# yc015/fully-automated-multi-heartbeat-echocardiography-video-segmentation-and-motion-tracking

Measured on AMD Instinct MI355X. Metric: 32f×112×112 clips/sec at 1/2/4/8 MI355X; Dice Δ vs CPU ref, higher is better.
Workload: dtype fp32

## Files before the change

### fully-automated-multi-heartbeat-echocardiography-video-segmentation-and-motion-tracking_amd/csrc/conv.hip

```cpp
#include <hip/hip_bf16.h>
#include <stdlib.h>
#include <string.h>

#include "common.h"

typedef __bf16 bf16x8 __attribute__((ext_vector_type(8)));

namespace {

__device__ inline bf16x8 pack_bf16x8(f32x4 a, f32x4 b) {
  return bf16x8{(__bf16)a[0], (__bf16)a[1], (__bf16)a[2], (__bf16)a[3],
                (__bf16)b[0], (__bf16)b[1], (__bf16)b[2], (__bf16)b[3]};
}

__device__ inline void split3_bf16x8(f32x4 a, f32x4 b, bf16x8& hi, bf16x8& mid, bf16x8& lo) {
  hi = pack_bf16x8(a, b);
#pragma unroll
  for (int e = 0; e < 4; ++e) {
    a[e] -= (float)hi[e];
    b[e] -= (float)hi[4 + e];
  }
  mid = pack_bf16x8(a, b);
#pragma unroll
  for (int e = 0; e < 4; ++e) {
// ... 916 lines not shown
    }
  };
  auto store_tiles = [&](int buf) {
#pragma unroll
    for (int i = 0; i < AL; ++i) As[buf][a_q[i]][a_r[i]] = ra[i];
#pragma unroll
    for (int i = 0; i < BL; ++i) {
      const int e = tid + i * NTH;
      if (e < B4) Bs[buf][e & 3][e >> 2] = rb[i];
    }
  };
  f32x4 acc[MT][NT];
#pragma unroll
  for (int i = 0; i < MT; ++i)
#pragma unroll
    for (int j = 0; j < NT; ++j) acc[i][j] = f32x4{0.f, 0.f, 0.f, 0.f};
  const int nk = p.Kp / 16;
  load_tiles(0);
  store_tiles(0);
  __syncthreads();
  int cur = 0;
  for (int kt = 0; kt < nk; ++kt) {
    const bool more = kt + 1 < nk;
    if (more) load_tiles((kt + 1) * 16);
    f32x4 a[MT], b[NT];
#pragma unroll
    for (int i = 0; i < MT; ++i) a[i] = As[cur][q][wid * 32 + i * 16 + l16];
#pragma unroll
    for (int j = 0; j < NT; ++j) b[j] = Bs[cur][q][j * 16 + l16];
#pragma unroll
    for (int kk = 0; kk < 4; ++kk)
#pragma unroll
      for (int i = 0; i < MT; ++i)
#pragma unroll
        for (int j = 0; j < NT; ++j)
          acc[i][j] = __builtin_amdgcn_mfma_f32_16x16x4f32(b[j][kk], a[i][kk], acc[i][j], 0, 0, 0);
    if (more) store_tiles(cur ^ 1);
    __syncthreads();
    cur ^= 1;
  }
  epilogue<MT, NT>(p, acc, m0 + wid * 32, n0, q, l16);
}


__device__ inline bf16x8 stem_bf16x8(f32x4 a, f32x4 b) {
  return bf16x8{(__bf16)a[0], (__bf16)a[1], (__bf16)a[2], (__bf16)a[3],
                (__bf16)b[0], (__bf16)b[1], (__bf16)b[2], (__bf16)b[3]};
}

__global__ __launch_bounds__(256) __attribute__((amdgpu_waves_per_eu(2))) void conv_stem_bf16(ConvParams p, int n_items) {
  constexpr int MT = 4, NT = 4, ROW = 7 * 64, IMG = 64 * ROW;
  __shared__ __align__(16) char ws[2 * IMG];
  const float* x = reinterpret_cast<const float*>(p.x);
  const char* w16 = reinterpret_cast<const char*>(p.w);
  const int tid = threadIdx.x, lane = tid & 63, wid = tid >> 6;
  const int q = lane >> 4, l16 = lane & 15;
  const int q8 = n_items >> 3, r8 = n_items & 7, x8 = blockIdx.x & 7;
  const int i_start = x8 < r8 ? x8 * (q8 + 1) : r8 * (q8 + 1) + (x8 - r8) * q8;
  const int i_end = i_start + q8 + (x8 < r8 ? 1 : 0);
  const int i_step = gridDim.x >> 3;
  if (i_start + (int)(blockIdx.x >> 3) >= i_end) return;
  for (int e = tid; e < 2 * 64 * 28; e += 256) {
    const int im = e / (64 * 28), r0 = e - im * (64 * 28);
    const int co = r0 / 28, r = r0 - co * 28, kh = r >> 2, sl = r & 3;
    *reinterpret_cast<uint4*>(ws + im * IMG + co * ROW + kh * 64 + ((sl ^ (co & 3)) << 4)) =
        *reinterpret_cast<const uint4*>(w16 + (size_t)im * 64 * 448 + (size_t)co * 448 + kh * 64 + sl * 16);
  }
  __syncthreads();
  const int b_rd = l16 * ROW + ((q ^ (l16 & 3)) << 4);
  f32x4 bv[NT];
#pragma unroll
  for (int j = 0; j < NT; ++j) bv[j] = *reinterpret_cast<const f32x4*>(p.bias + 16 * j + 4 * q);
#pragma unroll 1
  for (int item = i_start + (int)(blockIdx.x >> 3); item < i_end; item += i_step) {
    const int m0 = item * 256 + wid * 64;
    const float* rowp[MT];
    int hi0[MT], wi0[MT];
    bool live[MT];
#pragma unroll
    for (int i = 0; i < MT; ++i) {
      int m = m0 + 16 * i + l16;
      live[i] = m < p.M;
      if (!live[i]) m = 0;
      const int wo = m % p.Wo;
      m /= p.Wo;
      const int ho = m % p.Ho;
      const int nt = m / p.Ho;
      hi0[i] = 2 * ho - 3;
      wi0[i] = 2 * wo - 3 + 2 * q;
      rowp[i] = x + ((size_t)nt * p.Hi * p.Wi) * 4;
    }
    f32x4 acc[MT][NT];
#pragma unroll
    for (int i = 0; i < MT; ++i)
#pragma unroll
      for (int j = 0; j < NT; ++j) acc[i][j] = f32x4{0.f, 0.f, 0.f, 0.f};
#pragma unroll 1
    for (int kh = 0; kh < 7; ++kh) {
      bf16x8 ah[MT], al[MT], bh[NT], bl[NT];
#pragma unroll
      for (int i = 0; i < MT; ++i) {
        const int hi = hi0[i] + kh;
        const bool rok = live[i] && (unsigned)hi < (unsigned)p.Hi;
        const float* px = rowp[i] + ((size_t)hi * p.Wi + wi0[i]) * 4;
        f32x4 v0 = {0.f, 0.f, 0.f, 0.f}, v1 = {0.f, 0.f, 0.f, 0.f};
        if (rok && (unsigned)wi0[i] < (unsigned)p.Wi) v0 = *reinterpret_cast<const f32x4*>(px);
        if (rok && (unsigned)(wi0[i] + 1) < (unsigned)p.Wi) v1 = *reinterpret_cast<const f32x4*>(px + 4);
        ah[i] = stem_bf16x8(v0, v1);
        f32x4 r0, r1;
#pragma unroll
        for (int e = 0; e < 4; ++e) {
          r0[e] = v0[e] - (float)ah[i][e];
          r1[e] = v1[e] - (float)ah[i][4 + e];
        }
        al[i] = stem_bf16x8(r0, r1);
      }
#pragma unroll
      for (int j = 0; j < NT; ++j) {
        bh[j] = *reinterpret_cast<const bf16x8*>(ws + j * 16 * ROW + kh * 64 + b_rd);
        bl[j] = *reinterpret_cast<const bf16x8*>(ws + IMG + j * 16 * ROW + kh * 64 + b_rd);
      }
#pragma unroll
      for (int j = 0; j < NT; ++j)
#pragma unroll
        for (int i = 0; i < MT; ++i) {
          acc[i][j] = __builtin_amdgcn_mfma_f32_16x16x32_bf16(bl[j], ah[i], acc[i][j], 0, 0, 0);
          acc[i][j] = __builtin_amdgcn_mfma_f32_16x16x32_bf16(bh[j], al[i], acc[i][j], 0, 0, 0);
          acc[i][j] = __builtin_amdgcn_mfma_f32_16x16x32_bf16(bh[j], ah[i], acc[i][j], 0, 0, 0);
        }
    }
    __bf16* y = reinterpret_cast<__bf16*>(p.y);
#pragma unroll
    for (int i = 0; i < MT; ++i) {
      if (!live[i]) continue;
      const size_t m = (size_t)m0 + 16 * i + l16;
#pragma unroll
      for (int j = 0; j < NT; ++j) {
        const int n = 16 * j + 4 * q;
        f32x4 v = acc[i][j] + bv[j];
#pragma unroll
        for (int e = 0; e < 4; ++e) v[e] = relu1(v[e]);
        *reinterpret_cast<bf16x4*>(y + m * 64 + n) = bf16x4{(__bf16)v[0], (__bf16)v[1], (__bf16)v[2], (__bf16)v[3]};
      }
    }
  }
}

bool dma_buf_ok(const ConvParams& p, size_t es) {
  if ((p.vflags & CLASFV_VARIANT_NO_DMA_BUF) || es != 2) return false;
  const size_t lim = (size_t)1 << 31;
  const size_t vox = (size_t)p.N * p.Ti * p.Hi * p.Wi;
  const size_t padpix = ((size_t)p.pt * p.Hi + p.ph) * p.Wi + p.pw;
  return p.KT * p.KH * p.KW <= 32 && (vox + padpix) * p.Cin * es < lim && (!p.x2 || vox * p.Cin2 * es < lim) &&
         (size_t)p.Cout * p.Kp * es < lim;
}

bool dma_w_ok_(const ConvParams& p) {
  if (p.vflags & CLASFV_VARIANT_NO_DMA_W) return false;
  if (!p.in_bf16 || p.stem || p.n_split > 1 || !dma_buf_ok(p, 2)) return false;
  return p.Cin % 64 == 0 && (!p.x2 || p.Cin2 % 64 == 0) && p.Kp == p.K && p.Kp % 64 == 0;
}

template <int MT, int NT, int S>
hipError_t launch_dma_w(const ConvParams& p, hipStream_t s) {
  constexpr int BM = 64 * MT, BN = 16 * NT;
  const int mt = (p.M + BM - 1) / BM, nt = (p.Cout + BN - 1) / BN;
  const DmaDivs dv{fast_div(p.Wo), fast_div(p.Ho), fast_div(p.To), fast_div(nt)};
  CLASFV_LAUNCH((conv_dma_w<MT, NT, S>), dim3(mt * nt), dim3(256), 0, s, p, nt, dv);
  return hipGetLastError();
}

template <typename T, int MT, int NT, int S>
hipError_t launch_dma(const ConvParams& p, hipStream_t s) {
  constexpr int BM = 64 * MT, BN = 16 * NT;
  const int mt = (p.M + BM - 1) / BM, nt = (p.Cout + BN - 1) / BN;
  const DmaDivs dv{fast_div(p.Wo), fast_div(p.Ho), fast_div(p.To), fast_div(nt)};
  const int n_split = p.n_split > 1 ? p.n_split : 1;
  if constexpr (sizeof(T) == 2 && MT == 2)
    if (dma_w_ok_(p)) return launch_dma_w<MT, NT, 2>(p, s);
  if (dma_buf_ok(p, sizeof(T)))
    CLASFV_LAUNCH((conv_dma<T, MT, NT, S, true>), dim3(mt * nt * n_split), dim3(256), 0, s, p, nt, dv);
  else
    CLASFV_LAUNCH((conv_dma<T, MT, NT, S>), dim3(mt * nt * n_split), dim3(256), 0, s, p, nt, dv);
  if (n_split > 1) return launch_split_sum(p, s);
  return hipGetLastError();
}

bool dma_x3_buf_ok(const ConvParams& p, int rows_alloc) {
  if (p.vflags & CLASFV_VARIANT_NO_DMA_BUF) return false;
  const size_t lim = (size_t)1 << 31;
  const size_t vox = (size_t)p.N * p.Ti * p.Hi * p.Wi;
  const size_t padpix = ((size_t)p.pt * p.Hi + p.ph) * p.Wi + p.pw;
  const int npairs = (p.Kp / 16 + 1) / 2;
  return p.KT * p.KH * p.KW <= 31 && (vox + padpix) * p.Cin * 4 < lim && (!p.x2 || vox * p.Cin2 * 4 < lim) &&
         (size_t)rows_alloc * npairs * 192 < lim;
}

template <int MT, int NT, int S, int WN = 1>
hipError_t launch_dma_x3_t(const ConvParams& p, hipStream_t s) {
  constexpr int BM = 64 * MT, BN = 16 * NT;
  const int mt = (p.M + BM - 1) / BM, nt = (p.Cout + BN - 1) / BN;
  const DmaDivs dv{fast_div(p.Wo), fast_div(p.Ho), fast_div(p.To), fast_div(nt)};
  const int n_split = p.n_split > 1 ? p.n_split : 1;
  const dim3 grid(mt * nt * n_split);
  const int ef = n_split > 1 ? 0 : (p.res ? 1 : 0) | (p.relu ? 2 : 0) | (p.y_c8 ? 4 : 0);
  switch (dma_x3_buf_ok(p, nt * BN) ? ef + 8 : ef) {
    case 0: CLASFV_LAUNCH((conv_dma_x3<MT, NT, S, WN, 0>), grid, dim3(256), 0, s, p, nt, dv); break;
    case 1: CLASFV_LAUNCH((conv_dma_x3<MT, NT, S, WN, 1>), grid, dim3(256), 0, s, p, nt, dv); break;
    case 2: CLASFV_LAUNCH((conv_dma_x3<MT, NT, S, WN, 2>), grid, dim3(256), 0, s, p, nt, dv); break;
    case 3: CLASFV_LAUNCH((conv_dma_x3<MT, NT, S, WN, 3>), grid, dim3(256), 0, s, p, nt, dv); break;
    case 8: CLASFV_LAUNCH((conv_dma_x3<MT, NT, S, WN, 0, 0, true>), grid, dim3(256), 0, s, p, nt, dv); break;
    case 9: CLASFV_LAUNCH((conv_dma_x3<MT, NT, S, WN, 1, 0, true>), grid, dim3(256), 0, s, p, nt, dv); break;
    case 10: CLASFV_LAUNCH((conv_dma_x3<MT, NT, S, WN, 2, 0, true>), grid, dim3(256), 0, s, p, nt, dv); break;
    case 11: CLASFV_LAUNCH((conv_dma_x3<MT, NT, S, WN, 3, 0, true>), grid, dim3(256), 0, s, p, nt, dv); break;
    default:
      if (ef >= 8 || ef < 4) return hipErrorInvalidValue;
      if (dma_x3_buf_ok(p, nt * BN))
        CLASFV_LAUNCH((conv_dma_x3<MT, NT, S, WN, -1, 0, true>), grid, dim3(256), 0, s, p, nt, dv);
      else
        CLASFV_LAUNCH((conv_dma_x3<MT, NT, S, WN>), grid, dim3(256), 0, s, p, nt, dv);
      break;
  }
  if (n_split > 1) return launch_split_sum(p, s);
  return hipGetLastError();
}

template <int NT>
hipError_t launch_stem(const ConvParams& p, hipStream_t s) {
  if (p.Cin != 4 || p.KT != 1 || p.KH != 7 || p.KW != 7) return hipErrorInvalidValue;
  const int mt = (p.M + 127) / 128, nt = (p.Cout + 16 * NT - 1) / (16 * NT);
  CLASFV_LAUNCH((conv_stem_f32<NT>), dim3(mt * nt), dim3(256), 0, s, p, nt);
  return hipGetLastError();
}

#ifdef CLASFV_KNOCKOUTS
template <int NT, int KO>
hipError_t dma_ko_t(const ConvParams& p, hipStream_t s) {
  constexpr int BM = 128, BN = 16 * NT;
  const int mt = (p.M + BM - 1) / BM, nt = (p.Cout + BN - 1) / BN;
  const DmaDivs dv{fast_div(p.Wo), fast_div(p.Ho), fast_div(p.To), fast_div(nt)};
  CLASFV_LAUNCH((conv_dma<__bf16, 2, NT, 3, (KO & 1) == 0, KO & ~1>), dim3(mt * nt), dim3(256), 0, s, p, nt, dv);
  return hipGetLastError();
}
template <int NT>
hipError_t dma_ko_n(const ConvParams& p, int ko, hipStream_t s) {
  switch (ko) {
    case 0: return dma_ko_t<NT, 0>(p, s);
    case 1: return dma_ko_t<NT, 1>(p, s);
    case 4: return dma_ko_t<NT, 4>(p, s);
    case 8: return dma_ko_t<NT, 8>(p, s);
    case 16: return dma_ko_t<NT, 16>(p, s);
    case 12: return dma_ko_t<NT, 12>(p, s);
    case 28: return dma_ko_t<NT, 28>(p, s);
  }
  return hipErrorInvalidValue;
}
hipError_t dma_bf16_ko(const ConvParams& p, int bn, int ko, hipStream_t s) {
  if (ko == 100 || ko == 101) {
    if (!dma_w_ok_(p)) return hipErrorInvalidValue;
    switch (bn) {
      case 64: return ko == 100 ? launch_dma_w<2, 4, 2>(p, s) : launch_dma_w<2, 4, 3>(p, s);
      case 96: return ko == 100 ? launch_dma_w<2, 6, 2>(p, s) : launch_dma_w<2, 6, 3>(p, s);
      case 128: return ko == 100 ? launch_dma_w<2, 8, 2>(p, s) : launch_dma_w<2, 8, 3>(p, s);
    }
    return hipErrorInvalidValue;
  }
  if (!p.in_bf16 || p.n_split > 1) return hipErrorInvalidValue;
  switch (bn) {
    case 64: return dma_ko_n<4>(p, ko, s);
    case 96: return dma_ko_n<6>(p, ko, s);
    case 128: return dma_ko_n<8>(p, ko, s);
  }
  return hipErrorInvalidValue;
}
#endif

template <typename T>
hipError_t launch_typed(const ConvParams& p, int bn, hipStream_t s) {
  switch (bn) {
    case 48: return launch_dma<T, 2, 3, 3>(p, s);
    case 64: return launch_dma<T, 2, 4, 3>(p, s);
    case 80: return launch_dma<T, 2, 5, 3>(p, s);
    case 96: return launch_dma<T, 2, 6, 3>(p, s);
    case 128: return launch_dma<T, 2, 8, 3>(p, s);
    case 144: return launch_dma<T, 2, 9, 3>(p, s);
  }
  return hipErrorInvalidValue;
}

#ifdef CLASFV_KNOCKOUTS
hipError_t launch_bf16_m4(const ConvParams& p, int bn, hipStream_t s) {
  switch (bn) {
    case 48: return launch_dma<__bf16, 4, 3, 3>(p, s);
    case 64: return launch_dma<__bf16, 4, 4, 3>(p, s);
    case 80: return launch_dma<__bf16, 4, 5, 3>(p, s);
    case 96: return launch_dma<__bf16, 4, 6, 3>(p, s);
    case 128: return launch_dma<__bf16, 4, 8, 3>(p, s);
    case 144: return launch_dma<__bf16, 4, 9, 3>(p, s);
  }
  return hipErrorInvalidValue;
}
#endif

__global__ __launch_bounds__(256) __attribute__((amdgpu_waves_per_eu(2))) void conv_stem_x3(ConvParams p, int n_items) {
  constexpr int MT = 4, NT = 3, CO = 16 * NT, ROW = 7 * 64, IMG = CO * ROW;
  __shared__ __align__(16) char ws[3 * IMG];
  const float* x = reinterpret_cast<const float*>(p.x);
  const char* w16 = reinterpret_cast<const char*>(p.w);
  const int tid = threadIdx.x, lane = tid & 63, wid = tid >> 6;
  const int q = lane >> 4, l16 = lane & 15;
  const int q8 = n_items >> 3, r8 = n_items & 7, x8 = blockIdx.x & 7;
  const int i_start = x8 < r8 ? x8 * (q8 + 1) : r8 * (q8 + 1) + (x8 - r8) * q8;
  const int i_end = i_start + q8 + (x8 < r8 ? 1 : 0);
  const int i_step = gridDim.x >> 3;
  if (i_start + (int)(blockIdx.x >> 3) >= i_end) return;
  for (int e = tid; e < 3 * CO * 28; e += 256) {
    const int im = e / (CO * 28), r0 = e - im * (CO * 28);
    const int co = r0 / 28, r = r0 - co * 28, kh = r >> 2, sl = r & 3;
    *reinterpret_cast<uint4*>(ws + im * IMG + co * ROW + kh * 64 + ((sl ^ (co & 3)) << 4)) =
        *reinterpret_cast<const uint4*>(w16 + (size_t)im * CO * 448 + (size_t)co * 448 + kh * 64 + sl * 16);
  }
  __syncthreads();
  const int b_rd = l16 * ROW + ((q ^ (l16 & 3)) << 4);
#pragma unroll 1
  for (int item = i_start + (int)(blockIdx.x >> 3); item < i_end; item += i_step) {
  const int m0 = item * 256 + wid * 64;
  const float* rowp[MT];
  int hi0[MT], wi0[MT];
  bool live[MT];
#pragma unroll
  for (int i = 0; i < MT; ++i) {
    int m = m0 + 16 * i + l16;
    live[i] = m < p.M;
    if (!live[i]) m = 0;
    const int wo = m % p.Wo;
    m /= p.Wo;
    const int ho = m % p.Ho;
    const int nt = m / p.Ho;
    hi0[i] = 2 * ho - 3;
    wi0[i] = 2 * wo - 3 + 2 * q;
    rowp[i] = x + ((size_t)nt * p.Hi * p.Wi) * 4;
  }
  f32x4 acc[MT][NT];
#pragma unroll
  for (int i = 0; i < MT; ++i)
#pragma unroll
    for (int j = 0; j < NT; ++j) acc[i][j] = f32x4{0.f, 0.f, 0.f, 0.f};
#pragma unroll 1
  for (int kh = 0; kh < 7; ++kh) {
    bf16x8 ah[MT], am[MT], al[MT];
#pragma unroll
    for (int i = 0; i < MT; ++i) {
      const int hi = hi0[i] + kh;
      const bool rok = live[i] && (unsigned)hi < (unsigned)p.Hi;
      const float* px = rowp[i] + ((size_t)hi * p.Wi + wi0[i]) * 4;
      f32x4 v0 = {0.f, 0.f, 0.f, 0.f}, v1 = {0.f, 0.f, 0.f, 0.f};
      if (rok && (unsigned)wi0[i] < (unsigned)p.Wi) v0 = *reinterpret_cast<const f32x4*>(px);
      if (rok && (unsigned)(wi0[i] + 1) < (unsigned)p.Wi) v1 = *reinterpret_cast<const f32x4*>(px + 4);
      split3_bf16x8(v0, v1, ah[i], am[i], al[i]);
    }
#pragma unroll
    for (int j = 0; j < NT; ++j) {
      const bf16x8 bh = *reinterpret_cast<const bf16x8*>(ws + j * 16 * ROW + kh * 64 + b_rd);
      const bf16x8 bm = *reinterpret_cast<const bf16x8*>(ws + IMG + j * 16 * ROW + kh * 64 + b_rd);
      const bf16x8 bl = *reinterpret_cast<const bf16x8*>(ws + 2 * IMG + j * 16 * ROW + kh * 64 + b_rd);
#pragma unroll
      for (int i = 0; i < MT; ++i) {
        f32x4 c = acc[i][j];
        c = __builtin_amdgcn_mfma_f32_16x16x32_bf16(bl, ah[i], c, 0, 0, 0);
        c = __builtin_amdgcn_mfma_f32_16x16x32_bf16(bh, al[i], c, 0, 0, 0);
        c = __builtin_amdgcn_mfma_f32_16x16x32_bf16(bm, am[i], c, 0, 0, 0);
        c = __builtin_amdgcn_mfma_f32_16x16x32_bf16(bm, ah[i], c, 0, 0, 0);
        c = __builtin_amdgcn_mfma_f32_16x16x32_bf16(bh, am[i], c, 0, 0, 0);
        acc[i][j] = __builtin_amdgcn_mfma_f32_16x16x32_bf16(bh, ah[i], c, 0, 0, 0);
      }
    }
  }
  epilogue<MT, NT>(p, acc, m0, 0, q, l16);
  }
}

}

bool dma_w_ok(const ConvParams& p) { return dma_w_ok_(p); }

#ifdef CLASFV_KNOCKOUTS
hipError_t launch_dma_bf16_ko(const ConvParams& p, int bn, int ko, hipStream_t s) { return dma_bf16_ko(p, bn, ko, s); }
#endif

bool proj_x3_supported(const ConvParams& p) {
  if (p.vflags & CLASFV_VARIANT_NO_DMA_X3) return false;
  if (p.in_bf16 || p.out_bf16 || p.stem || p.x_c8 || p.y_c8 || p.n_split > 1) return false;
  if (p.KT != 1 || p.KH != 1 || p.KW != 1 || p.st != 1 || p.sh != 1 || p.sw != 1) return false;
  if (p.Cout != 64 || p.Cin % 32 || (p.x2 && p.Cin2 % 32)) return false;
  const int k = p.Cin + (p.x2 ? p.Cin2 : 0);
  if (p.Kp != k || k != 128) return false;
  return (size_t)p.M * (p.Cin > 64 ? p.Cin : 64) < ((size_t)1 << 31);
}

hipError_t launch_proj_x3(const ConvParams& p, hipStream_t s) {
  if (!proj_x3_supported(p)) return hipErrorInvalidValue;
  const int n_items = (p.M + 31) / 32;
  const int kb = p.Kp / 32;
  int blocks = 256;
  if (blocks * 4 > n_items) blocks = (n_items + 3) / 4;
  (void)kb;
  const int passes = (n_items + 4 * blocks - 1) / (4 * blocks);
  CLASFV_LAUNCH_P(passes, (conv_proj_x3<4, 3>), dim3(blocks), dim3(256), 0, s, p, n_items);
  return hipGetLastError();
}

bool dma_x3_supported(const ConvParams& p) {
  return !(p.vflags & CLASFV_VARIANT_NO_DMA_X3) && !p.in_bf16 && !p.out_bf16 && !p.stem && !p.x_c8 && !p.y_c8 &&
         p.Kp % 16 == 0 && p.Cin % 16 == 0 && (!p.x2 || p.Cin2 % 16 == 0) && p.Cout % 16 == 0;
}

int dma_x3_bn(int cout_p) {
  const int n16 = cout_p / 16;
  for (int c : {8, 6, 5, 4, 3})
    if (n16 % c == 0) return 16 * c;
  return 16 * (n16 % 2 == 0 ? 2 : 1);
}

hipError_t launch_dma_x3(const ConvParams& p, int bn, hipStream_t s) {
  if (!dma_x3_supported(p)) return hipErrorInvalidValue;
  switch (bn) {
    case 16: return launch_dma_x3_t<2, 1, 2>(p, s);
    case 32: return launch_dma_x3_t<2, 2, 2>(p, s);
    case 48: return launch_dma_x3_t<2, 3, 2>(p, s);
    case 64: return launch_dma_x3_t<2, 4, 2>(p, s);
    case 80: return launch_dma_x3_t<2, 5, 2>(p, s);
    case 96: return launch_dma_x3_t<2, 6, 2>(p, s);
    case 128: return launch_dma_x3_t<2, 8, 2>(p, s);
  }
  return hipErrorInvalidValue;
}

#ifdef CLASFV_KNOCKOUTS
hipError_t launch_dma_x3_cfg(const ConvParams& p, int mt, int nt, int S, hipStream_t s) {
  const int wn = getenv("CB_X3WN") ? atoi(getenv("CB_X3WN")) : 1;
  const int key = (wn == 2 ? 1000 : 0) + mt * 100 + nt * 10 + S;
  switch (key) {
    case 1242: return launch_dma_x3_t<2, 4, 2, 2>(p, s);
    case 1262: return launch_dma_x3_t<2, 6, 2, 2>(p, s);
    case 1282: return launch_dma_x3_t<2, 8, 2, 2>(p, s);
    case 1162: return launch_dma_x3_t<1, 6, 2, 2>(p, s);
    case 132: return launch_dma_x3_t<1, 3, 2>(p, s);
    case 133: return launch_dma_x3_t<1, 3, 3>(p, s);
    case 162: return launch_dma_x3_t<1, 6, 2>(p, s);
    case 163: return launch_dma_x3_t<1, 6, 3>(p, s);
    case 233: return launch_dma_x3_t<2, 3, 3>(p, s);
    case 243: return launch_dma_x3_t<2, 4, 3>(p, s);
    case 263: return launch_dma_x3_t<2, 6, 3>(p, s);
    case 432: return launch_dma_x3_t<4, 3, 2>(p, s);
    case 462: return launch_dma_x3_t<4, 6, 2>(p, s);
    case 152: return launch_dma_x3_t<1, 5, 2>(p, s);
    case 452: return launch_dma_x3_t<4, 5, 2>(p, s);
    case 253: return launch_dma_x3_t<2, 5, 3>(p, s);
    case 442: return launch_dma_x3_t<4, 4, 2>(p, s);
    case 482: return launch_dma_x3_t<4, 8, 2>(p, s);
    case 182: return launch_dma_x3_t<1, 8, 2>(p, s);
  }
  return launch_dma_x3(p, 16 * nt, s);
}

template <int NT, int KO>
static hipError_t dma_x3_ko_t(const ConvParams& p, hipStream_t s) {
  const int mt = (p.M + 127) / 128, nt = (p.Cout + 16 * NT - 1) / (16 * NT);
  const DmaDivs dv{fast_div(p.Wo), fast_div(p.Ho), fast_div(p.To), fast_div(nt)};
  CLASFV_LAUNCH((conv_dma_x3<2, NT, 2, 1, 2, (KO & 31), (KO & 32) != 0>), dim3(mt * nt), dim3(256), 0, s, p, nt, dv);
  return hipGetLastError();
}
hipError_t launch_dma_x3_ko(const ConvParams& p, int nt, int ko, hipStream_t s) {
  if (!dma_x3_supported(p) || p.res || !p.relu || p.y_c8 || p.n_split > 1) return hipErrorInvalidValue;
#define DX3KO(N)                                       \
  switch (ko) {                                        \
    case 0: return dma_x3_ko_t<N, 0>(p, s);             \
    case 1: return dma_x3_ko_t<N, 1>(p, s);             \
    case 2: return dma_x3_ko_t<N, 2>(p, s);             \
    case 4: return dma_x3_ko_t<N, 4>(p, s);             \
    case 8: return dma_x3_ko_t<N, 8>(p, s);             \
    case 16: return dma_x3_ko_t<N, 16>(p, s);           \
    case 31: return dma_x3_ko_t<N, 31>(p, s);           \
    case 32: return dma_x3_ko_t<N, 32>(p, s);           \
    case 33: return dma_x3_ko_t<N, 33>(p, s);           \
    case 34: return dma_x3_ko_t<N, 34>(p, s);           \
    case 36: return dma_x3_ko_t<N, 36>(p, s);           \
    case 40: return dma_x3_ko_t<N, 40>(p, s);           \
    case 48: return dma_x3_ko_t<N, 48>(p, s);           \
  }
  if (nt == 5) DX3KO(5)
  if (nt == 8) DX3KO(8)
#undef DX3KO
  return hipErrorInvalidValue;
}
#endif

void dma_x3_weight_image(const float* w, int cout_alloc, int Kp, uint16_t* out) {
  const int npairs = (Kp / 16 + 1) / 2;
  for (int n = 0; n < cout_alloc; ++n)
    for (int pr = 0; pr < npairs; ++pr)
      for (int sl = 0; sl < 32; ++sl) {
        const int q = sl >> 3, e = sl & 7;
        const int k = 32 * pr + (e < 4 ? 4 * q + e : 16 + 4 * q + (e - 4));
        double r = k < Kp ? (double)w[(size_t)n * Kp + k] : 0.0;
        for (int pc = 0; pc < 3; ++pc) {
          float f = (float)r;
          uint32_t u;
          memcpy(&u, &f, 4);
          const uint16_t b = (uint16_t)((u + 0x7fffu + ((u >> 16) & 1u)) >> 16);
          const uint32_t ub = (uint32_t)b << 16;
          float fb;
          memcpy(&fb, &ub, 4);
          out[(((size_t)pr * 3 + pc) * cout_alloc + n) * 32 + sl] = b;
          r -= fb;
        }
      }
}

size_t dma_x3_weight_elems(int cout_alloc, int Kp) { return (size_t)cout_alloc * ((Kp / 16 + 1) / 2) * 96; }

void conv_pick_tile(int M, int cout_p, int force_nt, int* mt_out, int* bn_out) {
  const int n16 = cout_p / 16;
  int nt = 3;
  for (int c : {9, 8, 6, 5, 4, 3})
    if (n16 % c == 0 && (force_nt <= 0 || c == force_nt)) {
      nt = c;
      break;
    }
  (void)M;
  *mt_out = 2;
  *bn_out = 16 * nt;
}

__global__ __launch_bounds__(256) void split_sum_kernel(const float* __restrict__ part, int n_split, long n4, int co4,
                                                        const float* __restrict__ bias, const float* res, int relu,
                                                        float* y) {
  const long i = (long)blockIdx.x * 256 + threadIdx.x;
  if (i >= n4) return;
  const f32x4* pp = reinterpret_cast<const f32x4*>(part);
  f32x4 v = pp[i];
  for (int k = 1; k < n_split; ++k) v += pp[(long)k * n4 + i];
  if (bias) v += reinterpret_cast<const f32x4*>(bias)[i % co4];
  if (res) v += reinterpret_cast<const f32x4*>(res)[i];
  if (relu)
#pragma unroll
    for (int c = 0; c < 4; ++c) v[c] = relu1(v[c]);
  reinterpret_cast<f32x4*>(y)[i] = v;
}

hipError_t launch_split_sum(const ConvParams& p, hipStream_t s) {
  if (p.in_bf16 || p.out_bf16 || p.y_c8 || p.Cout % 4 || !p.part) return hipErrorInvalidValue;
  const long n4 = (long)p.M * p.Cout / 4;
  CLASFV_LAUNCH(split_sum_kernel, dim3((unsigned)((n4 + 255) / 256)), dim3(256), 0, s, p.part, p.n_split, n4,
                p.Cout / 4, p.bias, (const float*)p.res, p.relu, (float*)p.y);
  return hipGetLastError();
}

int dma_split_for(const ConvParams& p, int mt) {
  if (p.in_bf16 || p.out_bf16 || p.y_c8 || p.stem || mt != 2 || (p.vflags & CLASFV_VARIANT_NO_SPLIT_K)) return 1;
  if ((long)p.To * p.Ho * p.Wo > 256 || p.Kp / 16 < 4 * 16) return 1;
  return 4;
}

hipError_t launch_conv(const ConvParams& p, int mt, int bn, hipStream_t s) {
#ifdef CLASFV_KNOCKOUTS
  if (mt == 4 && p.in_bf16 && !p.stem) return launch_bf16_m4(p, bn, s);
#endif
  if (mt != 2) return hipErrorInvalidValue;
  if (p.stem) {
    if (bn == 48) return launch_stem<3>(p, s);
    if (bn == 64) return launch_stem<4>(p, s);
    return hipErrorInvalidValue;
  }
  return p.in_bf16 ? launch_typed<__bf16>(p, bn, s) : launch_typed<float>(p, bn, s);
}

__global__ void pack_input_kernel(const float* __restrict__ x, float* __restrict__ y, int N, int T, int HW) {
  const size_t per = (size_t)T * HW;
  const size_t total = (size_t)N * per;
  for (size_t i = blockIdx.x * (size_t)blockDim.x + threadIdx.x; i < total; i += (size_t)gridDim.x * blockDim.x) {
    const size_t n = i / per, r = i - n * per;
    const float* src = x + n * 3 * per + r;
    f32x4 v = {src[0], src[per], src[2 * per], 0.f};
    reinterpret_cast<f32x4*>(y)[i] = v;
  }
}

hipError_t launch_pack_input(const float* x, float* y, int N, int T, int HW, hipStream_t s) {
  const size_t total = (size_t)N * T * HW;
  int blocks = (int)((total + 255) / 256);
  if (blocks > 4096) blocks = 4096;
  const size_t lanes = (size_t)blocks * 256;
  const long passes = (long)((total + lanes - 1) / lanes);
  CLASFV_LAUNCH_P(passes, pack_input_kernel, dim3(blocks), dim3(256), 0, s, x, y, N, T, HW);
  return hipGetLastError();
}

bool stem_bf16_supported(const ConvParams& p) {
  return p.stem && p.out_bf16 && p.Cin == 4 && p.Cout == 64 && p.KT == 1 && p.KH == 7 && p.KW == 7 && p.st == 1 &&
         p.sh == 2 && p.sw == 2 && p.pt == 0 && p.ph == 3 && p.pw == 3 && p.relu && !p.res && p.bias &&
         p.To == p.Ti && (size_t)p.M < ((size_t)1 << 31);
}

bool stem_x3_supported(const ConvParams& p) {
  return !(p.vflags & CLASFV_VARIANT_NO_STEM_X3) && p.stem && !p.out_bf16 && !p.in_bf16 && p.Cin == 4 &&
         p.Cout == 48 && p.KT == 1 && p.KH == 7 && p.KW == 7 && p.st == 1 && p.sh == 2 && p.sw == 2 && p.pt == 0 &&
         p.ph == 3 && p.pw == 3 && !p.res && !p.x_c8 && p.To == p.Ti && (size_t)p.M < ((size_t)1 << 31);
}

hipError_t launch_stem_x3(const ConvParams& p, hipStream_t s) {
  if (!stem_x3_supported(p)) return hipErrorInvalidValue;
  const int n_items = (int)((p.M + 255) / 256);
  const int grid = n_items >= 1024 ? 512 : (n_items + 7) / 8 * 8;
  const int passes = (n_items + grid - 1) / grid;
  CLASFV_LAUNCH_P(passes, conv_stem_x3, dim3(grid), dim3(256), 0, s, p, n_items);
  return hipGetLastError();
}

hipError_t launch_stem_bf16(const ConvParams& p, hipStream_t s) {
  if (!stem_bf16_supported(p)) return hipErrorInvalidValue;
  const int n_items = (int)((p.M + 255) / 256);
  const int grid = n_items >= 1024 ? 512 : (n_items + 7) / 8 * 8;
  const int passes = (n_items + grid - 1) / grid;
  CLASFV_LAUNCH_P(passes, conv_stem_bf16, dim3(grid), dim3(256), 0, s, p, n_items);
  return hipGetLastError();
}
```

Baseline: 1449.

## Software-pipeline stem x3 input row loads and use fast division

Restructures the stem conv kernel so the next kernel row (and the next item's first row) is loaded from global memory while the current row is split and fed to MFMAs, using clamped unconditional loads with masking after. Integer div/mod for output coordinate decode is replaced by precomputed fast-division magic numbers, and the epilogue is specialized at compile time on relu/c8 output flags. This aims to hide global load latency behind matrix math, at the cost of higher register pressure from the double-buffered rows and a fully unrolled kh loop.

```diff
diff --git a/fully-automated-multi-heartbeat-echocardiography-video-segmentation-and-motion-tracking_amd/csrc/conv.hip b/fully-automated-multi-heartbeat-echocardiography-video-segmentation-and-motion-tracking_amd/csrc/conv.hip
--- a/fully-automated-multi-heartbeat-echocardiography-video-segmentation-and-motion-tracking_amd/csrc/conv.hip
+++ b/fully-automated-multi-heartbeat-echocardiography-video-segmentation-and-motion-tracking_amd/csrc/conv.hip
@@ -1242,13 +1242,118 @@
 }
 #endif
 
-__global__ __launch_bounds__(256) __attribute__((amdgpu_waves_per_eu(2))) void conv_stem_x3(ConvParams p, int n_items) {
+__device__ __forceinline__ void stem_x3_items(const ConvParams& p, const DmaDivs& dv, const char* ws, int item, int i_end,
+                                              int i_step) {
   constexpr int MT = 4, NT = 3, CO = 16 * NT, ROW = 7 * 64, IMG = CO * ROW;
+  constexpr int PS = 4;
+  const float* x = reinterpret_cast<const float*>(p.x);
+  const int lane = threadIdx.x & 63, wid = threadIdx.x >> 6;
+  const int q = lane >> 4, l16 = lane & 15;
+  const size_t frame = (size_t)p.Hi * p.Wi * PS;
+  const int b_rd = l16 * ROW + ((q ^ (l16 & 3)) << 4);
+  const float* fp[MT];
+  int hi0[MT], o0[MT], o1[MT];
+  auto locate = [&](int it) {
+#pragma unroll
+    for (int i = 0; i < MT; ++i) {
+      int m = it * 256 + wid * 64 + 16 * i + l16;
+      const bool live = m < p.M;
+      if (!live) m = 0;
+      const int mw = fdiv(m, dv.wo), wo = m - mw * p.Wo;
+      const int nt = fdiv(mw, dv.ho), ho = mw - nt * p.Ho;
+      hi0[i] = 2 * ho - 3;
+      const int wi = 2 * wo - 3 + 2 * q;
+      o0[i] = live && (unsigned)wi < (unsigned)p.Wi ? wi * PS : -1;
+      o1[i] = live && (unsigned)(wi + 1) < (unsigned)p.Wi ? (wi + 1) * PS : -1;
+      fp[i] = x + (size_t)nt * frame;
+    }
+  };
+  auto load_row = [&](int kh, f32x4(&r)[MT][2]) {
+#pragma unroll
+    for (int i = 0; i < MT; ++i) {
+      const int hc = min(max(hi0[i] + kh, 0), p.Hi - 1);
+      const float* row = fp[i] + (size_t)hc * p.Wi * PS;
+      const int a0 = max(o0[i], 0), a1 = max(o1[i], 0);
+      r[i][0] = *reinterpret_cast<const f32x4*>(row + a0);
+      r[i][1] = *reinterpret_cast<const f32x4*>(row + a1);
+    }
+  };
+  auto split_row = [&](int kh, const f32x4(&r)[MT][2], bf16x8(&ah)[MT], bf16x8(&am)[MT], bf16x8(&al)[MT]) {
+    const f32x4 z = {0.f, 0.f, 0.f, 0.f};
+#pragma unroll
+    for (int i = 0; i < MT; ++i) {
+      const bool rok = (unsigned)(hi0[i] + kh) < (unsigned)p.Hi;
+      split3_bf16x8(rok && o0[i] >= 0 ? r[i][0] : z, rok && o1[i] >= 0 ? r[i][1] : z, ah[i], am[i], al[i]);
+    }
+  };
+  f32x4 cur[MT][2], nxt[MT][2];
+  locate(item);
+  load_row(0, cur);
+#pragma unroll 1
+  for (; item < i_end; item += i_step) {
+    const int m0 = item * 256 + wid * 64;
+    f32x4 acc[MT][NT];
+#pragma unroll
+    for (int i = 0; i < MT; ++i)
+#pragma unroll
+      for (int j = 0; j < NT; ++j) acc[i][j] = f32x4{0.f, 0.f, 0.f, 0.f};
+#pragma unroll
+    for (int kh = 0; kh < 7; ++kh) {
+      bf16x8 ah[MT], am[MT], al[MT];
+      bool more = true;
+      if (kh < 6) {
+        load_row(kh + 1, nxt);
+        __builtin_amdgcn_sched_barrier(0);
+        split_row(kh, cur, ah, am, al);
+      } else {
+        split_row(kh, cur, ah, am, al);
+        more = item + i_step < i_end;
+        if (more) {
+          locate(item + i_step);
+          load_row(0, nxt);
+        }
+        __builtin_amdgcn_sched_barrier(0);
+      }
+#pragma unroll
+      for (int j = 0; j < NT; ++j) {
+        const bf16x8 bh = *reinterpret_cast<const bf16x8*>(ws + j * 16 * ROW + kh * 64 + b_rd);
+        const bf16x8 bm = *reinterpret_cast<const bf16x8*>(ws + IMG + j * 16 * ROW + kh * 64 + b_rd);
+        const bf16x8 bl = *reinterpret_cast<const bf16x8*>(ws + 2 * IMG + j * 16 * ROW + kh * 64 + b_rd);
+#pragma unroll
+        for (int i = 0; i < MT; ++i) {
+          f32x4 c = acc[i][j];
+          c = __builtin_amdgcn_mfma_f32_16x16x32_bf16(bl, ah[i], c, 0, 0, 0);
+          c = __builtin_amdgcn_mfma_f32_16x16x32_bf16(bh, al[i], c, 0, 0, 0);
+          c = __builtin_amdgcn_mfma_f32_16x16x32_bf16(bm, am[i], c, 0, 0, 0);
+          c = __builtin_amdgcn_mfma_f32_16x16x32_bf16(bm, ah[i], c, 0, 0, 0);
+          c = __builtin_amdgcn_mfma_f32_16x16x32_bf16(bh, am[i], c, 0, 0, 0);
+          acc[i][j] = __builtin_amdgcn_mfma_f32_16x16x32_bf16(bh, ah[i], c, 0, 0, 0);
+        }
+      }
+      if (more) {
+#pragma unroll
+        for (int i = 0; i < MT; ++i) cur[i][0] = nxt[i][0], cur[i][1] = nxt[i][1];
+      }
+    }
+    if (p.y_c8) {
+      if (p.relu)
+        epilogue<MT, NT, 6>(p, acc, m0, 0, q, l16);
+      else
+        epilogue<MT, NT, 4>(p, acc, m0, 0, q, l16);
+    } else {
+      if (p.relu)
+        epilogue<MT, NT, 2>(p, acc, m0, 0, q, l16);
+      else
+        epilogue<MT, NT, 0>(p, acc, m0, 0, q, l16);
+    }
+  }
+}
+
+__global__ __launch_bounds__(256) __attribute__((amdgpu_waves_per_eu(2))) void conv_stem_x3(ConvParams p, int n_items, DmaDivs dv) {
+  constexpr int NT = 3, CO = 16 * NT, ROW = 7 * 64, IMG = CO * ROW;
   __shared__ __align__(16) char ws[3 * IMG];
-  const float* x = reinterpret_cast<const float*>(p.x);
   const char* w16 = reinterpret_cast<const char*>(p.w);
-  const int tid = threadIdx.x, lane = tid & 63, wid = tid >> 6;
-  const int q = lane >> 4, l16 = lane & 15;
+  const int tid = threadIdx.x;
   const int q8 = n_items >> 3, r8 = n_items & 7, x8 = blockIdx.x & 7;
   const int i_start = x8 < r8 ? x8 * (q8 + 1) : r8 * (q8 + 1) + (x8 - r8) * q8;
   const int i_end = i_start + q8 + (x8 < r8 ? 1 : 0);
@@ -1261,63 +1366,8 @@
         *reinterpret_cast<const uint4*>(w16 + (size_t)im * CO * 448 + (size_t)co * 448 + kh * 64 + sl * 16);
   }
   __syncthreads();
-  const int b_rd = l16 * ROW + ((q ^ (l16 & 3)) << 4);
-#pragma unroll 1
-  for (int item = i_start + (int)(blockIdx.x >> 3); item < i_end; item += i_step) {
-  const int m0 = item * 256 + wid * 64;
-  const float* rowp[MT];
-  int hi0[MT], wi0[MT];
-  bool live[MT];
-#pragma unroll
-  for (int i = 0; i < MT; ++i) {
-    int m = m0 + 16 * i + l16;
-    live[i] = m < p.M;
-    if (!live[i]) m = 0;
-    const int wo = m % p.Wo;
-    m /= p.Wo;
-    const int ho = m % p.Ho;
-    const int nt = m / p.Ho;
-    hi0[i] = 2 * ho - 3;
-    wi0[i] = 2 * wo - 3 + 2 * q;
-    rowp[i] = x + ((size_t)nt * p.Hi * p.Wi) * 4;
-  }
-  f32x4 acc[MT][NT];
-#pragma unroll
-  for (int i = 0; i < MT; ++i)
-#pragma unroll
-    for (int j = 0; j < NT; ++j) acc[i][j] = f32x4{0.f, 0.f, 0.f, 0.f};
-#pragma unroll 1
-  for (int kh = 0; kh < 7; ++kh) {
-    bf16x8 ah[MT], am[MT], al[MT];
-#pragma unroll
-    for (int i = 0; i < MT; ++i) {
-      const int hi = hi0[i] + kh;
-      const bool rok = live[i] && (unsigned)hi < (unsigned)p.Hi;
-      const float* px = rowp[i] + ((size_t)hi * p.Wi + wi0[i]) * 4;
-      f32x4 v0 = {0.f, 0.f, 0.f, 0.f}, v1 = {0.f, 0.f, 0.f, 0.f};
-      if (rok && (unsigned)wi0[i] < (unsigned)p.Wi) v0 = *reinterpret_cast<const f32x4*>(px);
-      if (rok && (unsigned)(wi0[i] + 1) < (unsigned)p.Wi) v1 = *reinterpret_cast<const f32x4*>(px + 4);
-      split3_bf16x8(v0, v1, ah[i], am[i], al[i]);
-    }
-#pragma unroll
-    for (int j = 0; j < NT; ++j) {
-      const bf16x8 bh = *reinterpret_cast<const bf16x8*>(ws + j * 16 * ROW + kh * 64 + b_rd);
-      const bf16x8 bm = *reinterpret_cast<const bf16x8*>(ws + IMG + j * 16 * ROW + kh * 64 + b_rd);
-      const bf16x8 bl = *reinterpret_cast<const bf16x8*>(ws + 2 * IMG + j * 16 * ROW + kh * 64 + b_rd);
-#pragma unroll
-      for (int i = 0; i < MT; ++i) {
-        f32x4 c = acc[i][j];
-        c = __builtin_amdgcn_mfma_f32_16x16x32_bf16(bl, ah[i], c, 0, 0, 0);
-        c = __builtin_amdgcn_mfma_f32_16x16x32_bf16(bh, al[i], c, 0, 0, 0);
-        c = __builtin_amdgcn_mfma_f32_16x16x32_bf16(bm, am[i], c, 0, 0, 0);
-        c = __builtin_amdgcn_mfma_f32_16x16x32_bf16(bm, ah[i], c, 0, 0, 0);
-        c = __builtin_amdgcn_mfma_f32_16x16x32_bf16(bh, am[i], c, 0, 0, 0);
-        acc[i][j] = __builtin_amdgcn_mfma_f32_16x16x32_bf16(bh, ah[i], c, 0, 0, 0);
-      }
-    }
-  }
-  epilogue<MT, NT>(p, acc, m0, 0, q, l16);
-  }
+  const int first = i_start + (int)(blockIdx.x >> 3);
+  stem_x3_items(p, dv, ws, first, i_end, i_step);
 }
 
 }
@@ -1554,7 +1604,8 @@
   const int n_items = (int)((p.M + 255) / 256);
   const int grid = n_items >= 1024 ? 512 : (n_items + 7) / 8 * 8;
   const int passes = (n_items + grid - 1) / grid;
-  CLASFV_LAUNCH_P(passes, conv_stem_x3, dim3(grid), dim3(256), 0, s, p, n_items);
+  const DmaDivs dv{fast_div(p.Wo), fast_div(p.Ho), fast_div(p.To), fast_div(p.To)};
+  CLASFV_LAUNCH_P(passes, conv_stem_x3, dim3(grid), dim3(256), 0, s, p, n_items, dv);
   return hipGetLastError();
 }
 
```

After: 1437. About the same (-0.8%).
